# shaygong322/Mujoco-LIP-MPC-Simulation

Hardware: AMD Instinct MI355X
Metric: MPC solves/sec (batched scenarios), N=3 horizon 5-obstacle, 1->8 MI355X (higher is better)
Workload: dtype f64

## Files before the change

### mujoco-lip-mpc-simulation_amd/csrc/alipmpc.hip

```cpp
#include <hip/hip_runtime.h>

#include <atomic>
#include <cmath>
#include <cstdint>
#include <cstdio>
#include <cstdlib>
#include <cstring>
#include <map>
#include <mutex>
#include <string>
#include <type_traits>
#include <unordered_map>
#include <vector>

#include "../../include/alipmpc.h"

#ifndef ALIP_PART
#define ALIP_PART_HOST 1
#define ALIP_PART_N(k) 1
#else
#define ALIP_PART_HOST (ALIP_PART == 0)
#define ALIP_PART_N(k) (ALIP_PART == (k))
#endif

// ... 1534 lines not shown
#pragma unroll
        for (int q = 0; q < RPL; ++q) {
            const int r = lane + WAVE * q;
            if (r < mo4) {
                double* rq = rc + r;
                rq[0] = ck_put(sr[q]);
                rq[mo4] = ck_put(zl[q]);
                rq[2 * mo4] = ck_put(zu[q]);
                rq[3 * mo4] = ck_put(idl[q]);
                rq[4 * mo4] = ck_put(idu[q]);
                rq[5 * mo4] = ck_put(cr[q]);
                rq[6 * mo4] = ck_put(ra0[q]);
                rq[7 * mo4] = ck_put(ra1[q]);
#pragma unroll
                for (int i = 0; i < 4; ++i) rq[(8 + i) * mo4] = ck_put(rv[q][i]);
            }
        }
        double* rf = rc + ck_filt(mo4) + lane;
        if (lane < nf) {
            rf[0] = ck_put(fth0);
            rf[2 * WAVE] = ck_put(fph0);
        }
        if (lane + WAVE < nf) {
            rf[WAVE] = ck_put(fth1);
            rf[3 * WAVE] = ck_put(fph1);
        }
        if (lane < NG) rc[ck_vme(mo4) + lane] = ck_put(vme);
        const double sv[13] = {ck_put(mu), ck_put(f_cur), ck_put(lsum_cur), ck_put(theta_c), ck_put(dw_last),
                               (double)nf, (double)it, (double)n_rest, (double)fail_it, (double)it_end,
                               theta_ok ? 1.0 : 0.0, rp ? 1.0 : 0.0, ck_put(theta_R)};
        double v = 0.0;
#pragma unroll
        for (int i = 0; i < 13; ++i) v = lane == i ? sv[i] : v;
        if (lane < 13) rc[ck_scal(mo4) + lane] = v;
        if (lane == 0) P.cont[cont_hdr(P.B) + k] = (uint32_t)b;
        if constexpr (sizeof(R) == 8) {
            if (lane == 0 && !to_team) {
                const int cls = rp ? CONT_PEND : CONT_REG;
                P.cont[cont_list(P.B, cls, (long long)atomicAdd(P.cont + cls, 1u))] = (uint32_t)k;
            }
        }
    };
    R phi_R = R(0.0);
    it = it0;
    for (;;) {
    if constexpr (RS) {
        if (rpend) {
            rpend = false;
#ifndef ALIP_NO_SETPRIO
            if (PR && role == 2) __builtin_amdgcn_s_setprio(3);
#endif
            STAMP(8);
            RELANE();
#pragma unroll
            for (int q = 0; q < RPL; ++q) {
                const int r = lane + WAVE * q;
                if (r < mo4) {
                    w.ry[r] = sr[q];
                    w.rsig[r] = zl[q];
                    w.rw[r] = zu[q];
                }
            }
            if (lane < NG) w.V[lane] = vme;
            wave_sync();
            const int rr = rfl(resto_wave<N, KSM, R>(wv, fth0, fph0, fth1, fph1, nf, mu, theta_R, it));
            STAMP(25);
            const int rcode = rr & 15;
            it = rr >> 4;
            RELANE();
            vme = lane < NG ? w.V[lane] : R(0.0);
            R lr = R(0.0);
#pragma unroll
            for (int q = 0; q < RPL; ++q) {
                const int r = lane + WAVE * q;
                if (r < mo4) {
                    sr[q] = w.ry[r];
                    zl[q] = w.rsig[r];
                    zu[q] = w.rw[r];
                }
#pragma unroll
                for (int i = 0; i < 4; ++i) rv[q][i] = w.V[gen_i(rg[q], i)];
                R o[6];
#pragma unroll
                for (int i = 0; i < 6; ++i) o[i] = w.obs6[6 * roi[q] + i];
                row_trans(rtype[q], rv[q], w.cst[K_GXG], w.cst[K_GYG], ra0[q], ra1[q]);
                cr[q] = row_value(rtype[q], rk[q], rv[q], ra0[q], ra1[q], o, CK);
                const R d1 = sr[q] - cl[q], d2 = cu[q] - sr[q];
                lr += llog(HL(q) ? (HU(q) ? d1 * d2 : d1) : (HU(q) ? d2 : R(1.0)));
                idl[q] = HL(q) ? rcp_nr(d1) : R(0.0);
                idu[q] = HU(q) ? rcp_nr(d2) : R(0.0);
                zl[q] = HL(q) ? fmin(fmax(zl[q], mu * R(1e-10) * idl[q]), R(1e10) * mu * idl[q]) : R(0.0);
                zu[q] = HU(q) ? fmin(fmax(zu[q], mu * R(1e-10) * idu[q]), R(1e10) * mu * idu[q]) : R(0.0);
            }
            lsum_cur = wsum(lr);
            f_cur = obj_sum<N, RPL>(cr, mr4);
            theta_ok = false;
            wave_sync();
            STAMP(24);
            if (rcode == RSW_INFEASIBLE || rcode == RSW_FAILED) {
                status = 2;
                break;
            }
            if (rcode == RSW_MAXITER) break;
        }
    }
    for (; it <= max_iter; ++it) {
        if ((ckpt_it > 0 && it == ckpt_it) || (TM && ckpt_tr > 0 && w.cst[K_NTR] >= R(ckpt_tr))) {
            put_record(TM && !(ckpt_it > 0 && it == ckpt_it), false);
            status = ST_CKPT;
            break;
        }
#ifndef ALIP_NO_SETPRIO
        if ((TM && tm < 0) || (PR && (role == 1 || (role == 2 && n_rest > 0))))
            ;
        else if (PR && role == 2 && it == 20)
            ;
        else if (it == 8)
            __builtin_amdgcn_s_setprio(1);
        else if (it == 14)
            __builtin_amdgcn_s_setprio(2);
        else if (it == 20)
            __builtin_amdgcn_s_setprio(3);
#endif
        R gl[NT];
        R jv[JC ? KSM : 1][NT];
        for (;;) {
            RELANE();
#pragma unroll
            for (int q = 0; q < RPL; ++q) {
                const int r = lane + WAVE * q;
                R o[6], cf[4], hx[6];
#pragma unroll
                for (int i = 0; i < 6; ++i) o[i] = w.obs6[6 * roi[q] + i];
                row_coef(rtype[q], rk[q], rv[q], ra0[q], ra1[q], o, CK, cf, hx);
                if (r < mo4) {
                    st4(w.rcoef + 4 * r, cf[0], cf[1], cf[2], cf[3]);
                    w.ry[r] = rtype[q] == R_OBJ ? -R(1.0) : zl[q] - zu[q];
                }
                if (rtype[q] == R_VBX) {
                    w.CT[rk[q] + 1] = ra1[q];
                    w.ST[rk[q] + 1] = ra0[q];
                }
                if (rtype[q] == R_OBJ) {
#pragma unroll
                    for (int i = 0; i < 6; ++i) w.hobj[6 * rk[q] + i] = hx[i];
                }
            }
            wave_sync();
// ... 153 lines not shown
                const R* Gb = G + 8 * kb * NCP;
                R gv[NT], sgv[NT];
#ifdef ALIP_S_DENSE
                const unsigned SCOLS = 0xFFu;
#else
                const unsigned SCOLS = (s & 1) ? 0x7Fu : 0x73u;
#endif
#pragma unroll
                for (int T = 0; T < NT; ++T) {
                    gv[T] = G[t * NCP + 16 * T + col];
                    R a = R(0.0);
#pragma unroll
                    for (int c2 = 0; c2 < 8; ++c2)
                        if ((SCOLS >> c2) & 1u) a += Srow[c2] * Gb[c2 * NCP + 16 * T + col];
                    sgv[T] = a;
                }
                auto* a = acc[s & 1];
                a[0] = Mfma<R>::run(gv[0], sgv[0], a[0]);
                if constexpr (NT == 2) {
                    a[1] = Mfma<R>::run(gv[0], sgv[1], a[1]);
                    a[2] = Mfma<R>::run(gv[1], sgv[1], a[2]);
                }
            }
#pragma unroll
            for (int T = 0; T < NT; ++T) rhsc[T] = gsum(pw[T]);
#pragma unroll
            for (int i = 0; i < 4; ++i) {
                const int row = Mfma<R>::row(g4, i);
                w.K[row * KLD + col] = acc[0][0][i] + acc[1][0][i];
                if constexpr (NT == 2) {
                    const R k1 = acc[0][1][i] + acc[1][1][i];
                    w.K[row * KLD + 16 + col] = k1;
                    w.K[(16 + col) * KLD + row] = k1;
                    w.K[(16 + row) * KLD + 16 + col] = acc[0][2][i] + acc[1][2][i];
                }
            }
        }
        wave_sync();
        STAMP(4);
        RELANE();
        R xv;
        bool fact_ok = true;
        {
            R rhs_l = R(0.0);
#pragma unroll
            for (int T = 0; T < NT; ++T) rhs_l = (lane < n && (lane >> 4) == T) ? rhsc[T] : rhs_l;
            if constexpr (GJ && GJ_REGS) {
                R a[n + 1];
                auto fill = [&](R dw) {
#pragma unroll
                    for (int j = 0; j < n; ++j) a[j] = (lane < n ? w.K[lane * KLD + j] : R(0.0)) + (lane == j ? dw : R(0.0));
                    a[n] = rhs_l + R(0.0);
                };
                fill(R(0));
                if (!gj_regs<n, R, gj_rb<RPL>>(a, lane)) {
                    R dw = dw_last == R(0.0) ? R(1e-4) : fmax(R(1e-20), dw_last / R(3.0));
                    for (;;) {
                        fill(dw);
                        if (gj_regs<n, R, gj_rb<RPL>>(a, lane)) break;
                        dw *= dw_last == R(0.0) ? R(100.0) : R(8.0);
                        if (dw > R(sizeof(R) == 8 ? 1e40 : 1e30)) {
                            fact_ok = false;
                            break;
                        }
                    }
                    dw_last = uni(dw);
                }
                xv = lane < n ? a[n] : R(0.0);
            } else if constexpr (GJ) {
                if (lane < n) w.K[lane * KLD + n] = rhs_l;
                wave_sync();
                gj_fill<n, KLD, GJLD>(w.K, w.S, lane, R(0));
                wave_sync();
                if (!gj_lds<n, GJLD>(w.S, lane)) {
                    R dw = dw_last == R(0.0) ? R(1e-4) : fmax(R(1e-20), dw_last / R(3.0));
                    for (;;) {
                        gj_fill<n, KLD, GJLD>(w.K, w.S, lane, dw);
                        wave_sync();
                        if (gj_lds<n, GJLD>(w.S, lane)) break;
                        dw *= dw_last == R(0.0) ? R(100.0) : R(8.0);
                        if (dw > R(sizeof(R) == 8 ? 1e40 : 1e30)) {
                            fact_ok = false;
                            break;
                        }
                    }
                    dw_last = uni(dw);
                }
                xv = lane < n ? w.S[lane * GJLD + n] : R(0.0);
            } else {
                R a[n];
                R myidg = R(1.0);
#pragma unroll
                for (int j = 0; j < n; ++j) a[j] = lane < n ? w.K[lane * KLD + j] : (lane == j ? R(1.0) : R(0.0));
                if (!chol_rows<n>(a, myidg, lane)) {
                    R dw = dw_last == R(0.0) ? R(1e-4) : fmax(R(1e-20), dw_last / R(3.0));
                    for (;;) {
#pragma unroll
                        for (int j = 0; j < n; ++j)
                            a[j] = (lane < n ? w.K[lane * KLD + j] : (lane == j ? R(1.0) : R(0.0))) +
                                   (lane == j ? dw : R(0.0));
                        if (chol_rows<n>(a, myidg, lane)) break;
                        dw *= dw_last == R(0.0) ? R(100.0) : R(8.0);
                        if (dw > R(sizeof(R) == 8 ? 1e40 : 1e30)) {
                            fact_ok = false;
                            break;
                        }
                    }
                    dw_last = uni(dw);
                }
                R acc = R(0.0), yv = R(0.0);
#pragma unroll
                for (int k = 0; k < n; ++k) {
                    const R yk = bcast((rhs_l - acc) * myidg, k);
                    yv = lane == k ? yk : yv;
                    acc += lane > k ? a[k] * yk : R(0.0);
                }
                wave_sync();
                if (lane < n) {
#pragma unroll
// ... 3298 lines not shown
```

### mujoco-lip-mpc-simulation_amd/csrc/resto_wave.inc

```
enum { RSW_OK = 0, RSW_INFEASIBLE = 1, RSW_MAXITER = 2, RSW_FAILED = 3 };

template <int N, int KSM, class R>
__device__ __forceinline__ int resto_wave(int wv, R fth0, R fph0, R fth1, R fph1, int nfo, R mu_o, R theta_R, int it)
{
    using D = Dim<N>;
    constexpr int n = D::n;
    constexpr int NT = D::NT;
    constexpr int NCP = D::NCP;
    constexpr int NG = D::NG;
    constexpr int KLD = D::KLD;
    constexpr int RPL = (4 * KSM + WAVE - 1) / WAVE;
    extern __shared__ __attribute__((aligned(16))) double smem[];
    const KP& P = *reinterpret_cast<const KP*>(smem);
    const R* G = reinterpret_cast<const R*>(smem + KP_DOUBLES);
    R* wsb = const_cast<R*>(G) + NG * NCP;
    int lane = lane_id();
    RSTAMP_DECL
    const int mr4 = rfl(P.mr4), mo4 = rfl(P.mo4), m_max = rfl(P.m_max), rps = rfl(P.rps);
    const int nc_max = rfl(P.nc_max), ne_max = rfl(P.ne_max), nobs = nc_max + ne_max;
    const int modi = rfl(P.modi), max_iter = rfl(P.max_iter);
    WSS<N, R> w = carve_s<N, R>(wsb + (size_t)wv * wss_elems<N, R>(nc_max, ne_max, mr4, mo4), nc_max, ne_max, mr4, mo4);
    const int nc_sel = w.nsel[0], ne_sel = w.nsel[1];
    const R rho = R(1000.0), tol = w.cst[K_TOL];
    const R gth = R(1e-5), gph = R(1e-8), sth = R(1.1), sph = R(2.3), eta = R(1e-8), gal = R(0.05);
    int g4 = lane >> 4, col = lane & 15;
#define RS_RELANE()                                                                                               \
    do {                                                                                                          \
        RELAUNDER(lane);                                                                                          \
        g4 = lane >> 4;                                                                                           \
        col = lane & 15;                                                                                          \
        for (int q_ = 0; q_ < RPL; ++q_) {                                                                        \
            RELAUNDER(rtype[q_]);                                                                                 \
            RELAUNDER(rk[q_]);                                                                                    \
            RELAUNDER(roi[q_]);                                                                                   \
            RELAUNDER(rg[q_]);                                                                                    \
            RELAUNDER(cl[q_]);                                                                                    \
            RELAUNDER(cu[q_]);                                                                                    \
        }                                                                                                         \
    } while (0)
#define RCK load_rowk(w.cst)
    int rtype[RPL], rk[RPL], roi[RPL];
    uint32_t rg[RPL];
    R cl[RPL], cu[RPL], rv[RPL][4], rdv[RPL][4], ra0[RPL], ra1[RPL], cr[RPL];
    R sr[RPL], vl[RPL], vu[RPL], pp[RPL], nn[RPL], zp[RPL], zn[RPL], yv[RPL], s0[RPL], zl0[RPL], zu0[RPL];
    R mu = mu_o, nbl = R(0), mal = R(0);
#pragma unroll
    for (int q = 0; q < RPL; ++q) {
        const int r = lane + WAVE * q;
        RowInfo ri;
        ri.type = R_NONE; ri.k = 0; ri.slot = 0;
        if (r < m_max) {
            ri = decode_row(P, r, nc_sel, ne_sel);
        } else if (r >= mr4 && r < mr4 + N) {
            ri.type = R_OBJ;
            ri.k = r - mr4 + 1;
        }
        rtype[q] = ri.type;
        rk[q] = ri.k;
        roi[q] = ri.type == R_CIR ? ri.slot : (ri.type == R_ELP ? nc_max + ri.slot : 0);
        rg[q] = row_gens(ri.type, ri.k);
        const R clo = r < mr4 ? w.rclo[r] : R(-INFINITY), cuo = r < mr4 ? w.rcuo[r] : R(INFINITY);
        cl[q] = isfinite(clo) ? clo - R(1e-8) * fmax(R(1.0), fabs(clo)) : -INFINITY;
        cu[q] = isfinite(cuo) ? cuo + R(1e-8) * fmax(R(1.0), fabs(cuo)) : INFINITY;
        const bool isc = ri.type < R_NONE;
        sr[q] = r < mo4 && isc ? w.ry[r] : R(0);
        zl0[q] = r < mo4 && isc ? w.rsig[r] : R(0);
        zu0[q] = r < mo4 && isc ? w.rw[r] : R(0);
        s0[q] = sr[q];
#pragma unroll
        for (int i = 0; i < 4; ++i) {
            rv[q][i] = w.V[gen_i(rg[q], i)];
            rdv[q][i] = R(0);
        }
        R o[6];
#pragma unroll
        for (int i = 0; i < 6; ++i) o[i] = w.obs6[6 * roi[q] + i];
        row_trans(rtype[q], rv[q], w.cst[K_GXG], w.cst[K_GYG], ra0[q], ra1[q]);
        cr[q] = row_value(rtype[q], rk[q], rv[q], ra0[q], ra1[q], o, RCK);
        if (isc) {
            mu = fmax(mu, fabs(cr[q] - sr[q]));
            nbl += R(2) + (R)isfinite(cl[q]) + (R)isfinite(cu[q]);
            mal += R(1);
        }
    }
    mu = wmax(mu);
    nbl = wsum(nbl);
    mal = wsum(mal);
    const R xR = lane < n ? w.V[gp(lane / 3, lane % 3)] : R(0);
    const R d2 = lane < n ? R(1) / (fmax(R(1), fabs(xR)) * fmax(R(1), fabs(xR))) : R(0);
    R th0 = R(0);
#pragma unroll
    for (int q = 0; q < RPL; ++q) {
        const bool isc = rtype[q] < R_NONE;
        const R r_ = cr[q] - sr[q];
        const R a = (mu - rho * r_) / (R(2) * rho);
        const R sq = sqrt(a * a + mu * r_ / (R(2) * rho));
        const R nv = a >= R(0) ? a + sq : (mu * r_ / (R(2) * rho)) / (sq - a);
        nn[q] = isc ? nv : R(1);
        pp[q] = isc ? r_ + nv : R(1);
        zp[q] = isc ? mu / pp[q] : R(0);
        zn[q] = isc ? mu / nn[q] : R(0);
        vl[q] = isc && isfinite(cl[q]) ? fmin(rho, zl0[q]) : R(0);
        vu[q] = isc && isfinite(cu[q]) ? fmin(rho, zu0[q]) : R(0);
        yv[q] = R(0);
        if (isc) th0 += fabs(cr[q] - pp[q] + nn[q] - sr[q]);
    }
    th0 = wsum(th0);
    const R theta_max = R(1e4) * fmax(R(1), th0), theta_min = R(1e-4) * fmax(R(1), th0);
    R rft0 = INFINITY, rfp0 = INFINITY, rft1 = INFINITY, rfp1 = INFINITY;
    int nfr = 0;
    R dw_last = R(0);
    int code = RSW_OK;
    bool first = true;
    const int it_in = it;
    RSTAMP(0);
    for (;;) {
        RS_RELANE();
        R xc = lane < n ? w.V[gp(lane / 3, lane % 3)] : R(0);
        if (!first) {
            R tho = R(0), lso = R(0);
#pragma unroll
            for (int q = 0; q < RPL; ++q) {
                if (rtype[q] < R_NONE) tho += fabs(cr[q] - sr[q]);
                const R d1 = sr[q] - cl[q], d2_ = cu[q] - sr[q];
                lso += llog(isfinite(cl[q]) ? (isfinite(cu[q]) ? d1 * d2_ : d1) : (isfinite(cu[q]) ? d2_ : R(1.0)));
            }
            wsum_pair(tho, lso);
            const R fo = obj_sum<N, RPL>(cr, mr4);
            const R pho = fo - mu_o * lso;
            bool acc = isfinite(pho) && tho <= R(0.9) * theta_R;
            if (acc) {
                const bool b0 = lane < nfo && !(tho < fth0 || pho < fph0);
                const bool b1 = lane + WAVE < nfo && !(tho < fth1 || pho < fph1);
                acc = __ballot(b0 || b1) == 0ull;
            }
            if (acc) {
                const R tau = uni(fmax(R(0.99), R(1) - mu_o));
                R dzl[RPL], dzu[RPL], ad = R(1);
#pragma unroll
                for (int q = 0; q < RPL; ++q) {
                    const bool hl = rtype[q] < R_NONE && isfinite(cl[q]), hu = rtype[q] < R_NONE && isfinite(cu[q]);
                    const R e1 = s0[q] - cl[q], e2 = cu[q] - s0[q];
                    dzl[q] = hl ? mu_o / e1 - zl0[q] - zl0[q] / e1 * (sr[q] - s0[q]) : R(0);
                    dzu[q] = hu ? mu_o / e2 - zu0[q] + zu0[q] / e2 * (sr[q] - s0[q]) : R(0);
                    if (hl && dzl[q] < R(0)) ad = fmin(ad, -tau * zl0[q] / dzl[q]);
                    if (hu && dzu[q] < R(0)) ad = fmin(ad, -tau * zu0[q] / dzu[q]);
                }
                ad = wmin(ad);
                R zmax = R(0);
#pragma unroll
                for (int q = 0; q < RPL; ++q) {
                    zl0[q] += ad * dzl[q];
                    zu0[q] += ad * dzu[q];
                    zmax = fmax(zmax, fmax(zl0[q], zu0[q]));
                }
                zmax = wmax(zmax);
                if (zmax > R(1000)) {
#pragma unroll
                    for (int q = 0; q < RPL; ++q) {
                        zl0[q] = rtype[q] < R_NONE && isfinite(cl[q]) ? R(1) : R(0);
                        zu0[q] = rtype[q] < R_NONE && isfinite(cu[q]) ? R(1) : R(0);
                    }
                }
                code = RSW_OK;
                break;
            }
        }
        first = false;
        RSTAMP(1);
#pragma unroll
        for (int q = 0; q < RPL; ++q) {
            const int r = lane + WAVE * q;
            R o[6], cf[4], hx[6];
#pragma unroll
            for (int i = 0; i < 6; ++i) o[i] = w.obs6[6 * roi[q] + i];
            row_coef(rtype[q], rk[q], rv[q], ra0[q], ra1[q], o, RCK, cf, hx);
            if (r < mo4) {
                const bool isc = rtype[q] < R_NONE;
                st4(w.rcoef + 4 * r, isc ? cf[0] : R(0), isc ? cf[1] : R(0), isc ? cf[2] : R(0), isc ? cf[3] : R(0));
                w.ry[r] = isc ? yv[q] : R(0);
            }
            if (rtype[q] == R_VBX) {
                w.CT[rk[q] + 1] = ra1[q];
                w.ST[rk[q] + 1] = ra0[q];
            }
            if (rtype[q] == R_OBJ) {
#pragma unroll
                for (int i = 0; i < 6; ++i) w.hobj[6 * rk[q] + i] = R(0);
            }
        }
        wave_sync();
        constexpr bool JCR = KSM * NT <= 16;
        R jv[JCR ? KSM : 1][NT];
        R gl[NT];
#pragma unroll
        for (int T = 0; T < NT; ++T) gl[T] = R(0);
#pragma unroll
        for (int s = 0; s < KSM; ++s) {
            const int r = 4 * s + g4;
            const uint32_t pk = w.rgen[r];
            R ca0, ca1, cb0, cb1;
            ld4(w.rcoef + 4 * r, ca0, ca1, cb0, cb1);
            const R y = w.ry[r];
#pragma unroll
            for (int T = 0; T < NT; ++T) {
                const int cc = 16 * T + col;
                const R j = ca0 * G[gen_i(pk, 0) * NCP + cc] + ca1 * G[gen_i(pk, 1) * NCP + cc] +
                            cb0 * G[gen_i(pk, 2) * NCP + cc] + cb1 * G[gen_i(pk, 3) * NCP + cc];
                if constexpr (JCR) jv[JCR ? s : 0][T] = j;
                gl[T] += j * y;
            }
        }
#pragma unroll
        for (int T = 0; T < NT; ++T) gl[T] = gsum(gl[T]);
        R glme = gl[0];
#pragma unroll
        for (int T = 1; T < NT; ++T) glme = (lane >> 4) == T ? gl[T] : glme;
// ... 12 lines not shown
                nz += fabs(zp[q]) + fabs(zn[q]) + fabs(vl[q]) + fabs(vu[q]);
                whi = fmax(whi, fmax(pp[q] * zp[q], nn[q] * zn[q]));
                wlo = fmin(wlo, fmin(pp[q] * zp[q], nn[q] * zn[q]));
                if (isfinite(cl[q])) {
                    whi = fmax(whi, dl * vl[q]);
                    wlo = fmin(wlo, dl * vl[q]);
                }
                if (isfinite(cu[q])) {
                    whi = fmax(whi, du * vu[q]);
                    wlo = fmin(wlo, du * vu[q]);
                }
            }
        }
        wsum_pair(nz, ny);
        wmax_pair(dual, prim);
        wmaxmin_pair(whi, wlo);
        const R sd = uni(fmax(R(100), (nz + ny) / (R(n) + mal * R(3))) / R(100));
        const R sc = uni(fmax(R(100), nz / fmax(R(1), nbl)) / R(100));
        const R base = fmax(dual / sd, prim);
        const R e0 = uni(fmax(base, fmax(fabs(whi), fabs(wlo)) / sc));
        if (e0 <= tol) {
            R viol = R(0);
#pragma unroll
            for (int q = 0; q < RPL; ++q) {
                const int r = lane + WAVE * q;
                if (r < mr4 && rtype[q] < R_NONE) {
                    if (isfinite(cl[q])) viol = fmax(viol, w.rclo[r] - cr[q]);
                    if (isfinite(cu[q])) viol = fmax(viol, cr[q] - w.rcuo[r]);
                }
            }
            viol = wmax(viol);
            code = viol > R(1e-4) ? RSW_INFEASIBLE : RSW_OK;
            break;
        }
        if (it >= max_iter) {
            code = RSW_MAXITER;
            break;
        }
        const R mu_prev = mu;
        for (int t = 0; t < 8; ++t) {
            const R cm = fmax(fabs(whi - mu), fabs(wlo - mu));
            if (fmax(base, cm / sc) <= R(10) * mu && mu > tol / R(11))
                mu = uni(fmax(tol / R(11), fmin(R(0.2) * mu, mu * sqrt(mu))));
            else
                break;
        }
        if (mu != mu_prev) {
            nfr = 0;
            zeta = uni(sqrt(mu));
            gxv = lane < n ? zeta * d2 * (xc - xR) - glme : R(0);
        }
        const R tau = uni(fmax(R(0.99), R(1) - mu));
        RSTAMP(3);
        R iD[RPL], bv[RPL], iSp[RPL], iSn[RPL], iSs[RPL];
#pragma unroll
        for (int q = 0; q < RPL; ++q) {
            const int r = lane + WAVE * q;
            const bool isc = rtype[q] < R_NONE;
            const R dl = sr[q] - cl[q], du = cu[q] - sr[q];
            const R ipv = rcp_nr(pp[q]), inv = rcp_nr(nn[q]);
            const R idl_ = isfinite(cl[q]) ? rcp_nr(dl) : R(0), idu_ = isfinite(cu[q]) ? rcp_nr(du) : R(0);
            iSp[q] = isc ? pp[q] * rcp_nr(zp[q]) : R(0);
            iSn[q] = isc ? nn[q] * rcp_nr(zn[q]) : R(0);
            iSs[q] = isc ? rcp_nr(vl[q] * idl_ + vu[q] * idu_) : R(0);
            const R mdl = mu * idl_, mdu = mu * idu_;
            const R rc = cr[q] - pp[q] + nn[q] - sr[q];
            iD[q] = isc ? rcp_nr(iSp[q] + iSn[q] + iSs[q]) : R(0);
            bv[q] = isc ? -rc + (-rho - yv[q] + mu * ipv) * iSp[q] - (-rho + yv[q] + mu * inv) * iSn[q] +
                              (-yv[q] + mdl - mdu) * iSs[q]
                        : R(0);
            if (r < mo4) {
                w.rsig[r] = iD[q];
                w.rw[r] = isc ? yv[q] + bv[q] * iD[q] : R(0);
            }
        }
        wave_sync();
        RS_RELANE();
        RSTAMP(4);
        if constexpr (16 * (N + 1) <= WAVE)
            hess_blocks_lanes<N, R>(w, lane, rps, nobs, modi);
        else
            hess_blocks<N, R>(w, lane, rps, nobs, modi);
        wave_sync();
        RS_RELANE();
        RSTAMP(5);
        R rhsc[NT];
        {
            constexpr int NA = NT * (NT + 1) / 2;
            typename Mfma<R>::acc acc[2][NA];
#pragma unroll
            for (int h = 0; h < 2; ++h)
#pragma unroll
                for (int i = 0; i < NA; ++i) acc[h][i] = typename Mfma<R>::acc{R(0), R(0), R(0), R(0)};
            R pw[NT];
#pragma unroll
            for (int T = 0; T < NT; ++T) pw[T] = R(0);
#pragma unroll
            for (int s = 0; s < KSM; ++s) {
                const int r = 4 * s + g4;
                const R sg = w.rsig[r], wr = w.rw[r];
                R j[NT];
                if constexpr (JCR) {
#pragma unroll
                    for (int T = 0; T < NT; ++T) j[T] = jv[JCR ? s : 0][T];
                } else {
                    const uint32_t pk = w.rgen[r];
                    R ca0, ca1, cb0, cb1;
                    ld4(w.rcoef + 4 * r, ca0, ca1, cb0, cb1);
#pragma unroll
                    for (int T = 0; T < NT; ++T) {
                        const int cc = 16 * T + col;
                        j[T] = ca0 * G[gen_i(pk, 0) * NCP + cc] + ca1 * G[gen_i(pk, 1) * NCP + cc] +
                               cb0 * G[gen_i(pk, 2) * NCP + cc] + cb1 * G[gen_i(pk, 3) * NCP + cc];
                    }
                }
#pragma unroll
                for (int T = 0; T < NT; ++T) pw[T] += j[T] * wr;
                auto* a = acc[s & 1];
                a[0] = Mfma<R>::run(j[0], sg * j[0], a[0]);
                if constexpr (NT == 2) {
                    a[1] = Mfma<R>::run(j[0], sg * j[1], a[1]);
// ... 4 lines not shown
            for (int s = 1; s < NG / 4; ++s) {
                const int t = 4 * s + g4;
                const int kb = t >> 3;
                const R* Srow = w.S + 64 * kb + 8 * (t & 7);
                const R* Gb = G + 8 * kb * NCP;
                R gv[NT], sgv[NT];
                const unsigned SCOLS = (s & 1) ? 0x7Fu : 0x73u;
#pragma unroll
                for (int T = 0; T < NT; ++T) {
                    gv[T] = G[t * NCP + 16 * T + col];
                    R a = R(0);
#pragma unroll
                    for (int c2 = 0; c2 < 8; ++c2)
                        if ((SCOLS >> c2) & 1u) a += Srow[c2] * Gb[c2 * NCP + 16 * T + col];
                    sgv[T] = a;
                }
                auto* a = acc[s & 1];
                a[0] = Mfma<R>::run(gv[0], sgv[0], a[0]);
                if constexpr (NT == 2) {
                    a[1] = Mfma<R>::run(gv[0], sgv[1], a[1]);
                    a[2] = Mfma<R>::run(gv[1], sgv[1], a[2]);
                }
            }
#pragma unroll
            for (int T = 0; T < NT; ++T) rhsc[T] = gsum(pw[T]);
#pragma unroll
            for (int i = 0; i < 4; ++i) {
                const int row = Mfma<R>::row(g4, i);
                w.K[row * KLD + col] = acc[0][0][i] + acc[1][0][i];
                if constexpr (NT == 2) {
                    const R k1 = acc[0][1][i] + acc[1][1][i];
                    w.K[row * KLD + 16 + col] = k1;
                    w.K[(16 + col) * KLD + row] = k1;
                    w.K[(16 + row) * KLD + 16 + col] = acc[0][2][i] + acc[1][2][i];
                }
            }
        }
        wave_sync();
        if (lane < n) w.K[lane * KLD + lane] += zeta * d2;
        wave_sync();
        R rhs_l = R(0);
#pragma unroll
        for (int T = 0; T < NT; ++T) rhs_l = (lane < n && (lane >> 4) == T) ? rhsc[T] : rhs_l;
        rhs_l = lane < n ? rhs_l - zeta * d2 * (xc - xR) : R(0);
        RSTAMP(6);
        R xv;
        if constexpr (n <= ALIP_GJ_MAX_N) {
            R a[n + 1];
            auto fill = [&](R dw) {
#pragma unroll
                for (int j = 0; j < n; ++j) a[j] = (lane < n ? w.K[lane * KLD + j] : R(0)) + (lane == j ? dw : R(0));
                a[n] = rhs_l + R(0);
            };
            fill(R(0));
            bool ok = gj_regs<n, R, gj_rb<RPL>>(a, lane);
            if (!ok) {
                R dw = dw_last == R(0) ? R(1e-4) : fmax(R(1e-20), dw_last / R(3));
                for (;;) {
                    fill(dw);
                    if (gj_regs<n, R, gj_rb<RPL>>(a, lane)) {
                        ok = true;
                        break;
                    }
                    dw *= dw_last == R(0) ? R(100) : R(8);
                    if (dw > R(sizeof(R) == 8 ? 1e40 : 1e30)) break;
                }
                dw_last = uni(dw);
            }
            if (!ok) {
                code = RSW_FAILED;
                break;
            }
            xv = lane < n ? a[n] : R(0);
        } else {
            R a[n];
            R myidg = R(1);
#pragma unroll
            for (int j = 0; j < n; ++j) a[j] = lane < n ? w.K[lane * KLD + j] : (lane == j ? R(1) : R(0));
            bool ok = chol_rows<n>(a, myidg, lane);
            if (!ok) {
                R dw = dw_last == R(0) ? R(1e-4) : fmax(R(1e-20), dw_last / R(3));
                for (;;) {
#pragma unroll
                    for (int j = 0; j < n; ++j)
                        a[j] = (lane < n ? w.K[lane * KLD + j] : (lane == j ? R(1) : R(0))) + (lane == j ? dw : R(0));
                    if (chol_rows<n>(a, myidg, lane)) {
                        ok = true;
                        break;
                    }
                    dw *= dw_last == R(0) ? R(100) : R(8);
                    if (dw > R(sizeof(R) == 8 ? 1e40 : 1e30)) break;
                }
                dw_last = uni(dw);
            }
            if (!ok) {
                code = RSW_FAILED;
                break;
            }
            R acc = R(0), yy = R(0);
#pragma unroll
            for (int k = 0; k < n; ++k) {
                const R yk = bcast((rhs_l - acc) * myidg, k);
                yy = lane == k ? yk : yy;
                acc += lane > k ? a[k] * yk : R(0);
            }
            wave_sync();
            if (lane < n) {
#pragma unroll
                for (int j = 0; j < n; ++j) w.K[lane * KLD + j] = j <= lane ? a[j] : R(0);
            }
            wave_sync();
            acc = R(0);
            xv = R(0);
#pragma unroll
            for (int i = n - 1; i >= 0; --i) {
                const R xi = bcast((yy - acc) * myidg, i);
                xv = lane == i ? xi : xv;
                acc += lane < i ? w.K[i * KLD + (lane & 31)] * xi : R(0);
            }
        }
        RS_RELANE();
        RSTAMP(7);
        {
            R v = R(0);
            if constexpr (dp_rows<n, NG, R>) {
                v = gdp_rows<n, NCP>(G, xv, lane < NG ? lane : 0);
            } else {
#pragma unroll
                for (int j = 0; j < n; ++j) v += G[(lane < NG ? lane : 0) * NCP + j] * bcast(xv, j);
            }
            if (lane < NG) w.dV[lane] = v;
        }
        wave_sync();
        R dy[RPL], dpv[RPL], dnv[RPL], ds[RPL], dzp[RPL], dzn[RPL], dvl[RPL], dvu[RPL];
        R ap = R(1), az = R(1), theta = R(0), lin = R(0), gpn = R(0);
#pragma unroll
        for (int q = 0; q < RPL; ++q) {
            const int r = lane + WAVE * q;
#pragma unroll
            for (int i = 0; i < 4; ++i) rdv[q][i] = w.dV[gen_i(rg[q], i)];
            R jd = R(0);
            if (r < mo4) {
                R ca0, ca1, cb0, cb1;
                ld4(w.rcoef + 4 * r, ca0, ca1, cb0, cb1);
                jd = ca0 * rdv[q][0] + ca1 * rdv[q][1] + cb0 * rdv[q][2] + cb1 * rdv[q][3];
            }
            const bool isc = rtype[q] < R_NONE, hl = isc && isfinite(cl[q]), hu = isc && isfinite(cu[q]);
            const R dl = sr[q] - cl[q], du = cu[q] - sr[q];
            const R ipv = rcp_nr(pp[q]), inv = rcp_nr(nn[q]);
            const R idl_ = hl ? rcp_nr(dl) : R(0), idu_ = hu ? rcp_nr(du) : R(0);
            const R mdl = mu * idl_, mdu = mu * idu_;
            dy[q] = isc ? (bv[q] - jd) * iD[q] : R(0);
            dpv[q] = isc ? (-rho - yv[q] + mu * ipv - dy[q]) * iSp[q] : R(0);
            dnv[q] = isc ? (-rho + yv[q] + mu * inv + dy[q]) * iSn[q] : R(0);
            ds[q] = isc ? (-yv[q] + mdl - mdu - dy[q]) * iSs[q] : R(0);
            dzp[q] = isc ? mu * ipv - zp[q] - zp[q] * ipv * dpv[q] : R(0);
            dzn[q] = isc ? mu * inv - zn[q] - zn[q] * inv * dnv[q] : R(0);
            dvl[q] = hl ? mdl - vl[q] - vl[q] * idl_ * ds[q] : R(0);
            dvu[q] = hu ? mdu - vu[q] + vu[q] * idu_ * ds[q] : R(0);
            if (isc) {
                if (dpv[q] < R(0)) ap = fmin(ap, -tau * pp[q] * rcp_nr(dpv[q]));
                if (dnv[q] < R(0)) ap = fmin(ap, -tau * nn[q] * rcp_nr(dnv[q]));
                if (dzp[q] < R(0)) az = fmin(az, -tau * zp[q] * rcp_nr(dzp[q]));
                if (dzn[q] < R(0)) az = fmin(az, -tau * zn[q] * rcp_nr(dzn[q]));
                theta += fabs(cr[q] - pp[q] + nn[q] - sr[q]);
                gpn += (rho - mu * ipv) * dpv[q] + (rho - mu * inv) * dnv[q] - (mdl - mdu) * ds[q];
                lin += rho * (pp[q] + nn[q]) - mu * llog(pp[q] * nn[q] * (hl ? (hu ? dl * du : dl) : (hu ? du : R(1))));
            }
            const R ids = rcp_nr(ds[q]);
            if (hl && ds[q] < R(0)) ap = fmin(ap, -tau * dl * ids);
            if (hu && ds[q] > R(0)) ap = fmin(ap, tau * du * ids);
            if (hl && dvl[q] < R(0)) az = fmin(az, -tau * vl[q] * rcp_nr(dvl[q]));
            if (hu && dvu[q] < R(0)) az = fmin(az, -tau * vu[q] * rcp_nr(dvu[q]));
        }
        const R ex = lane < n ? xc - xR : R(0);
        lin += R(0.5) * zeta * d2 * ex * ex;
        gpn += zeta * d2 * ex * xv;
        wmin_pair(ap, az);
        wsum_pair(theta, gpn);
        const R gphi = gpn;
        const R phi = wsum(lin);
        R amin;
        if (gphi < R(0)) {
            amin = fmin(gth, gph * theta / -gphi);
            if (theta <= theta_min) amin = fmin(amin, exp(sth * llog(theta) - sph * llog(-gphi)));
        } else {
            amin = gth;
        }
        amin *= gal;
        amin = uni(amin > R(0) ? amin : R(8.673617379884035e-19));
        RSTAMP(8);
        R al = ap;
        bool accepted = false, ftype = false;
        R ctr[RPL], ta0[RPL], ta1[RPL];
        const R dxl = lane < n ? xv : R(0);
        while (al >= amin) {
            R tht = R(0), lt = R(0);
            bool bad = false;
#pragma unroll
            for (int q = 0; q < RPL; ++q) {
                R vt[4];
#pragma unroll
                for (int i = 0; i < 4; ++i) vt[i] = fma(al, rdv[q][i], rv[q][i]);
                R o[6];
#pragma unroll
                for (int i = 0; i < 6; ++i) o[i] = w.obs6[6 * roi[q] + i];
                row_trans(rtype[q], vt, w.cst[K_GXG], w.cst[K_GYG], ta0[q], ta1[q]);
                ctr[q] = row_value(rtype[q], rk[q], vt, ta0[q], ta1[q], o, RCK);
                if (rtype[q] < R_NONE) {
                    const R pt = pp[q] + al * dpv[q], nt = nn[q] + al * dnv[q], st = sr[q] + al * ds[q];
                    tht += fabs(ctr[q] - pt + nt - st);
                    const R d1 = st - cl[q], d2_ = cu[q] - st;
                    if (!(pt > R(0)) || !(nt > R(0))) bad = true;
                    if (isfinite(cl[q]) && !(d1 > R(0))) bad = true;
                    if (isfinite(cu[q]) && !(d2_ > R(0))) bad = true;
                    lt += rho * (pt + nt) -
                          mu * llog(pt * nt * (isfinite(cl[q]) ? (isfinite(cu[q]) ? d1 * d2_ : d1)
                                                               : (isfinite(cu[q]) ? d2_ : R(1))));
                }
// ... 25 lines not shown
                    ftype = false;
                }
            }
            if (accepted) break;
            al = uni(al * R(0.5));
        }
        RSTAMP(9);
        if (!accepted) {
            code = RSW_FAILED;
            break;
        }
        if (!ftype && nfr < FILTER_CAP) {
            const R fvt = (R(1) - gth) * theta, fvp = phi - gph * theta;
            if ((nfr & (WAVE - 1)) == lane) {
                if (nfr < WAVE) {
                    rft0 = fvt;
                    rfp0 = fvp;
                } else {
                    rft1 = fvt;
                    rfp1 = fvp;
                }
            }
            nfr++;
        }
        if (lane < NG) w.V[lane] = fma(al, w.dV[lane], w.V[lane]);
#pragma unroll
        for (int q = 0; q < RPL; ++q) {
#pragma unroll
            for (int i = 0; i < 4; ++i) rv[q][i] = fma(al, rdv[q][i], rv[q][i]);
            ra0[q] = ta0[q];
            ra1[q] = ta1[q];
            cr[q] = ctr[q];
            if (rtype[q] < R_NONE) {
                pp[q] += al * dpv[q];
                nn[q] += al * dnv[q];
                sr[q] += al * ds[q];
                yv[q] += al * dy[q];
                zp[q] += az * dzp[q];
                zn[q] += az * dzn[q];
                vl[q] += az * dvl[q];
                vu[q] += az * dvu[q];
                const R ks = R(1e10);
                zp[q] = fmin(fmax(zp[q], mu / (ks * pp[q])), ks * mu / pp[q]);
                zn[q] = fmin(fmax(zn[q], mu / (ks * nn[q])), ks * mu / nn[q]);
                const R d1 = sr[q] - cl[q], d2_ = cu[q] - sr[q];
                vl[q] = isfinite(cl[q]) ? fmin(fmax(vl[q], mu / (ks * d1)), ks * mu / d1) : R(0);
                vu[q] = isfinite(cu[q]) ? fmin(fmax(vu[q], mu / (ks * d2_)), ks * mu / d2_) : R(0);
            }
        }
        wave_sync();
        ++it;
        RSTAMP(10);
    }
    wave_sync();
#pragma unroll
    for (int q = 0; q < RPL; ++q) {
        const int r = lane + WAVE * q;
        if (r < mo4) {
            w.ry[r] = sr[q];
            w.rsig[r] = zl0[q];
            w.rw[r] = zu0[q];
        }
    }
    wave_sync();
    RSTAMP(11);
    RSTAMP_FLUSH(it - it_in);
    return (it << 4) | code;
#undef RS_RELANE
#undef RCK
}
```

Measured before the change: 7.835 million.

## Pass restoration row state in registers instead of round-tripping through LDS

The restoration-phase routine now takes the caller's per-row register arrays (types, bounds, slacks, multipliers, constraint values) by reference. This drops the LDS write-back and re-read of slacks and multipliers and the row decoding and constraint evaluation it repeated on entry. On a successful return it also hands back the barrier-log sum and objective, so the caller skips recomputing them. It also reuses reciprocals computed in the matrix build for the step direction, makes the acceptance test compute the log-barrier only when the theta test passes, and merges the regularised factorisation retry into one loop, at the cost of higher register pressure in the inlined routine.

Measured after the change: 7.942 million (median of 6 runs). +1.4%, better.

```diff
diff --git a/mujoco-lip-mpc-simulation_amd/csrc/alipmpc.hip b/mujoco-lip-mpc-simulation_amd/csrc/alipmpc.hip
--- a/mujoco-lip-mpc-simulation_amd/csrc/alipmpc.hip
+++ b/mujoco-lip-mpc-simulation_amd/csrc/alipmpc.hip
@@ -1610,48 +1610,44 @@
 #endif
             STAMP(8);
             RELANE();
-#pragma unroll
-            for (int q = 0; q < RPL; ++q) {
-                const int r = lane + WAVE * q;
-                if (r < mo4) {
-                    w.ry[r] = sr[q];
-                    w.rsig[r] = zl[q];
-                    w.rw[r] = zu[q];
-                }
-            }
             if (lane < NG) w.V[lane] = vme;
             wave_sync();
-            const int rr = rfl(resto_wave<N, KSM, R>(wv, fth0, fph0, fth1, fph1, nf, mu, theta_R, it));
+            R lso = R(0.0), fro = R(0.0);
+            const int rr = rfl(resto_wave<N, KSM, R>(wv, fth0, fph0, fth1, fph1, nf, mu, theta_R, it, rtype, rk, roi, rg,
+                                                     cl, cu, rv, ra0, ra1, cr, sr, zl, zu, lso, fro));
             STAMP(25);
             const int rcode = rr & 15;
             it = rr >> 4;
             RELANE();
             vme = lane < NG ? w.V[lane] : R(0.0);
-            R lr = R(0.0);
+            if (rcode == RSW_OK_ORIG) {
+                lsum_cur = lso;
+                f_cur = fro;
+            } else {
+                R lr = R(0.0);
+#pragma unroll
+                for (int q = 0; q < RPL; ++q) {
+#pragma unroll
+                    for (int i = 0; i < 4; ++i) rv[q][i] = w.V[gen_i(rg[q], i)];
+                    R o[6];
+#pragma unroll
+                    for (int i = 0; i < 6; ++i) o[i] = w.obs6[6 * roi[q] + i];
+                    row_trans(rtype[q], rv[q], w.cst[K_GXG], w.cst[K_GYG], ra0[q], ra1[q]);
+                    cr[q] = row_value(rtype[q], rk[q], rv[q], ra0[q], ra1[q], o, CK);
+                    const R d1 = sr[q] - cl[q], d2 = cu[q] - sr[q];
+                    lr += llog(HL(q) ? (HU(q) ? d1 * d2 : d1) : (HU(q) ? d2 : R(1.0)));
+                }
+                lsum_cur = wsum(lr);
+                f_cur = obj_sum<N, RPL>(cr, mr4);
+            }
 #pragma unroll
             for (int q = 0; q < RPL; ++q) {
-                const int r = lane + WAVE * q;
-                if (r < mo4) {
-                    sr[q] = w.ry[r];
-                    zl[q] = w.rsig[r];
-                    zu[q] = w.rw[r];
-                }
-#pragma unroll
-                for (int i = 0; i < 4; ++i) rv[q][i] = w.V[gen_i(rg[q], i)];
-                R o[6];
-#pragma unroll
-                for (int i = 0; i < 6; ++i) o[i] = w.obs6[6 * roi[q] + i];
-                row_trans(rtype[q], rv[q], w.cst[K_GXG], w.cst[K_GYG], ra0[q], ra1[q]);
-                cr[q] = row_value(rtype[q], rk[q], rv[q], ra0[q], ra1[q], o, CK);
                 const R d1 = sr[q] - cl[q], d2 = cu[q] - sr[q];
-                lr += llog(HL(q) ? (HU(q) ? d1 * d2 : d1) : (HU(q) ? d2 : R(1.0)));
                 idl[q] = HL(q) ? rcp_nr(d1) : R(0.0);
                 idu[q] = HU(q) ? rcp_nr(d2) : R(0.0);
                 zl[q] = HL(q) ? fmin(fmax(zl[q], mu * R(1e-10) * idl[q]), R(1e10) * mu * idl[q]) : R(0.0);
                 zu[q] = HU(q) ? fmin(fmax(zu[q], mu * R(1e-10) * idu[q]), R(1e10) * mu * idu[q]) : R(0.0);
             }
-            lsum_cur = wsum(lr);
-            f_cur = obj_sum<N, RPL>(cr, mr4);
             theta_ok = false;
             wave_sync();
             STAMP(24);
@@ -1911,6 +1907,23 @@
                     for (int j = 0; j < n; ++j) a[j] = (lane < n ? w.K[lane * KLD + j] : R(0.0)) + (lane == j ? dw : R(0.0));
                     a[n] = rhs_l + R(0.0);
                 };
+                if constexpr (RS) {
+                    R dw = R(0);
+                    for (;;) {
+                        fill(dw);
+                        if (gj_regs<n, R, gj_rb<RPL>>(a, lane)) break;
+                        if (dw == R(0)) {
+                            dw = dw_last == R(0.0) ? R(1e-4) : fmax(R(1e-20), dw_last / R(3.0));
+                        } else {
+                            dw *= dw_last == R(0.0) ? R(100.0) : R(8.0);
+                            if (dw > R(sizeof(R) == 8 ? 1e40 : 1e30)) {
+                                fact_ok = false;
+                                break;
+                            }
+                        }
+                    }
+                    if (dw != R(0)) dw_last = uni(dw);
+                } else {
                 fill(R(0));
                 if (!gj_regs<n, R, gj_rb<RPL>>(a, lane)) {
                     R dw = dw_last == R(0.0) ? R(1e-4) : fmax(R(1e-20), dw_last / R(3.0));
@@ -1924,6 +1937,7 @@
                         }
                     }
                     dw_last = uni(dw);
+                }
                 }
                 xv = lane < n ? a[n] : R(0.0);
             } else if constexpr (GJ) {
diff --git a/mujoco-lip-mpc-simulation_amd/csrc/resto_wave.inc b/mujoco-lip-mpc-simulation_amd/csrc/resto_wave.inc
--- a/mujoco-lip-mpc-simulation_amd/csrc/resto_wave.inc
+++ b/mujoco-lip-mpc-simulation_amd/csrc/resto_wave.inc
@@ -1,26 +1,28 @@
-enum { RSW_OK = 0, RSW_INFEASIBLE = 1, RSW_MAXITER = 2, RSW_FAILED = 3 };
+enum { RSW_OK = 0, RSW_INFEASIBLE = 1, RSW_MAXITER = 2, RSW_FAILED = 3, RSW_OK_ORIG = 4 };
 
-template <int N, int KSM, class R>
-__device__ __forceinline__ int resto_wave(int wv, R fth0, R fph0, R fth1, R fph1, int nfo, R mu_o, R theta_R, int it)
+template <int N, int KSM, class R, int RPL>
+__device__ __forceinline__ int resto_wave(int wv, R fth0, R fph0, R fth1, R fph1, int nfo, R mu_o, R theta_R, int it,
+                                          int (&rtype)[RPL], int (&rk)[RPL], int (&roi)[RPL], uint32_t (&rg)[RPL],
+                                          R (&cl)[RPL], R (&cu)[RPL], R (&rv)[RPL][4], R (&ra0)[RPL], R (&ra1)[RPL],
+                                          R (&cr)[RPL], R (&sr)[RPL], R (&zl0)[RPL], R (&zu0)[RPL], R& lsum_o, R& f_o)
 {
+    static_assert(RPL == (4 * KSM + WAVE - 1) / WAVE, "one row group per 64 rows");
     using D = Dim<N>;
     constexpr int n = D::n;
     constexpr int NT = D::NT;
     constexpr int NCP = D::NCP;
     constexpr int NG = D::NG;
     constexpr int KLD = D::KLD;
-    constexpr int RPL = (4 * KSM + WAVE - 1) / WAVE;
     extern __shared__ __attribute__((aligned(16))) double smem[];
     const KP& P = *reinterpret_cast<const KP*>(smem);
     const R* G = reinterpret_cast<const R*>(smem + KP_DOUBLES);
     R* wsb = const_cast<R*>(G) + NG * NCP;
     int lane = lane_id();
     RSTAMP_DECL
-    const int mr4 = rfl(P.mr4), mo4 = rfl(P.mo4), m_max = rfl(P.m_max), rps = rfl(P.rps);
+    const int mr4 = rfl(P.mr4), mo4 = rfl(P.mo4), rps = rfl(P.rps);
     const int nc_max = rfl(P.nc_max), ne_max = rfl(P.ne_max), nobs = nc_max + ne_max;
     const int modi = rfl(P.modi), max_iter = rfl(P.max_iter);
     WSS<N, R> w = carve_s<N, R>(wsb + (size_t)wv * wss_elems<N, R>(nc_max, ne_max, mr4, mo4), nc_max, ne_max, mr4, mo4);
-    const int nc_sel = w.nsel[0], ne_sel = w.nsel[1];
     const R rho = R(1000.0), tol = w.cst[K_TOL];
     const R gth = R(1e-5), gph = R(1e-8), sth = R(1.1), sph = R(2.3), eta = R(1e-8), gal = R(0.05);
     int g4 = lane >> 4, col = lane & 15;
@@ -39,53 +41,18 @@
         }                                                                                                         \
     } while (0)
 #define RCK load_rowk(w.cst)
-    int rtype[RPL], rk[RPL], roi[RPL];
-    uint32_t rg[RPL];
-    R cl[RPL], cu[RPL], rv[RPL][4], rdv[RPL][4], ra0[RPL], ra1[RPL], cr[RPL];
-    R sr[RPL], vl[RPL], vu[RPL], pp[RPL], nn[RPL], zp[RPL], zn[RPL], yv[RPL], s0[RPL], zl0[RPL], zu0[RPL];
-    R mu = mu_o, nbl = R(0), mal = R(0);
+    R rdv[RPL][4];
+    R vl[RPL], vu[RPL], pp[RPL], nn[RPL], zp[RPL], zn[RPL], yv[RPL], s0[RPL];
+    const R mal = w.cst[K_MACT], nbl = R(2) * mal + w.cst[K_NBL];
+    R mu = mu_o;
 #pragma unroll
     for (int q = 0; q < RPL; ++q) {
-        const int r = lane + WAVE * q;
-        RowInfo ri;
-        ri.type = R_NONE; ri.k = 0; ri.slot = 0;
-        if (r < m_max) {
-            ri = decode_row(P, r, nc_sel, ne_sel);
-        } else if (r >= mr4 && r < mr4 + N) {
-            ri.type = R_OBJ;
-            ri.k = r - mr4 + 1;
-        }
-        rtype[q] = ri.type;
-        rk[q] = ri.k;
-        roi[q] = ri.type == R_CIR ? ri.slot : (ri.type == R_ELP ? nc_max + ri.slot : 0);
-        rg[q] = row_gens(ri.type, ri.k);
-        const R clo = r < mr4 ? w.rclo[r] : R(-INFINITY), cuo = r < mr4 ? w.rcuo[r] : R(INFINITY);
-        cl[q] = isfinite(clo) ? clo - R(1e-8) * fmax(R(1.0), fabs(clo)) : -INFINITY;
-        cu[q] = isfinite(cuo) ? cuo + R(1e-8) * fmax(R(1.0), fabs(cuo)) : INFINITY;
-        const bool isc = ri.type < R_NONE;
-        sr[q] = r < mo4 && isc ? w.ry[r] : R(0);
-        zl0[q] = r < mo4 && isc ? w.rsig[r] : R(0);
-        zu0[q] = r < mo4 && isc ? w.rw[r] : R(0);
         s0[q] = sr[q];
 #pragma unroll
-        for (int i = 0; i < 4; ++i) {
-            rv[q][i] = w.V[gen_i(rg[q], i)];
-            rdv[q][i] = R(0);
-        }
-        R o[6];
-#pragma unroll
-        for (int i = 0; i < 6; ++i) o[i] = w.obs6[6 * roi[q] + i];
-        row_trans(rtype[q], rv[q], w.cst[K_GXG], w.cst[K_GYG], ra0[q], ra1[q]);
-        cr[q] = row_value(rtype[q], rk[q], rv[q], ra0[q], ra1[q], o, RCK);
-        if (isc) {
-            mu = fmax(mu, fabs(cr[q] - sr[q]));
-            nbl += R(2) + (R)isfinite(cl[q]) + (R)isfinite(cu[q]);
-            mal += R(1);
-        }
+        for (int i = 0; i < 4; ++i) rdv[q][i] = R(0);
+        if (rtype[q] < R_NONE) mu = fmax(mu, fabs(cr[q] - sr[q]));
     }
     mu = wmax(mu);
-    nbl = wsum(nbl);
-    mal = wsum(mal);
     const R xR = lane < n ? w.V[gp(lane / 3, lane % 3)] : R(0);
     const R d2 = lane < n ? R(1) / (fmax(R(1), fabs(xR)) * fmax(R(1), fabs(xR))) : R(0);
     R th0 = R(0);
@@ -118,21 +85,30 @@
         RS_RELANE();
         R xc = lane < n ? w.V[gp(lane / 3, lane % 3)] : R(0);
         if (!first) {
-            R tho = R(0), lso = R(0);
-#pragma unroll
-            for (int q = 0; q < RPL; ++q) {
+            R tho = R(0);
+#pragma unroll
+            for (int q = 0; q < RPL; ++q)
                 if (rtype[q] < R_NONE) tho += fabs(cr[q] - sr[q]);
-                const R d1 = sr[q] - cl[q], d2_ = cu[q] - sr[q];
-                lso += llog(isfinite(cl[q]) ? (isfinite(cu[q]) ? d1 * d2_ : d1) : (isfinite(cu[q]) ? d2_ : R(1.0)));
-            }
-            wsum_pair(tho, lso);
-            const R fo = obj_sum<N, RPL>(cr, mr4);
-            const R pho = fo - mu_o * lso;
-            bool acc = isfinite(pho) && tho <= R(0.9) * theta_R;
+            tho = wsum(tho);
+            bool acc = tho <= R(0.9) * theta_R;
             if (acc) {
-                const bool b0 = lane < nfo && !(tho < fth0 || pho < fph0);
-                const bool b1 = lane + WAVE < nfo && !(tho < fth1 || pho < fph1);
-                acc = __ballot(b0 || b1) == 0ull;
+                R lso = R(0);
+#pragma unroll
+                for (int q = 0; q < RPL; ++q) {
+                    const R d1 = sr[q] - cl[q], d2_ = cu[q] - sr[q];
+                    lso += llog(isfinite(cl[q]) ? (isfinite(cu[q]) ? d1 * d2_ : d1) : (isfinite(cu[q]) ? d2_ : R(1.0)));
+                }
+                lso = wsum(lso);
+                const R fo = obj_sum<N, RPL>(cr, mr4);
+                const R pho = fo - mu_o * lso;
+                lsum_o = lso;
+                f_o = fo;
+                acc = isfinite(pho);
+                if (acc) {
+                    const bool b0 = lane < nfo && !(tho < fth0 || pho < fph0);
+                    const bool b1 = lane + WAVE < nfo && !(tho < fth1 || pho < fph1);
+                    acc = __ballot(b0 || b1) == 0ull;
+                }
             }
             if (acc) {
                 const R tau = uni(fmax(R(0.99), R(1) - mu_o));
@@ -162,7 +138,7 @@
                         zu0[q] = rtype[q] < R_NONE && isfinite(cu[q]) ? R(1) : R(0);
                     }
                 }
-                code = RSW_OK;
+                code = RSW_OK_ORIG;
                 break;
             }
         }
@@ -281,21 +257,23 @@
         }
         const R tau = uni(fmax(R(0.99), R(1) - mu));
         RSTAMP(3);
-        R iD[RPL], bv[RPL], iSp[RPL], iSn[RPL], iSs[RPL];
+        R iD[RPL], bv[RPL], iSp[RPL], iSn[RPL], iSs[RPL], ipv[RPL], inv[RPL], idl_[RPL], idu_[RPL];
 #pragma unroll
         for (int q = 0; q < RPL; ++q) {
             const int r = lane + WAVE * q;
             const bool isc = rtype[q] < R_NONE;
             const R dl = sr[q] - cl[q], du = cu[q] - sr[q];
-            const R ipv = rcp_nr(pp[q]), inv = rcp_nr(nn[q]);
-            const R idl_ = isfinite(cl[q]) ? rcp_nr(dl) : R(0), idu_ = isfinite(cu[q]) ? rcp_nr(du) : R(0);
+            ipv[q] = rcp_nr(pp[q]);
+            inv[q] = rcp_nr(nn[q]);
+            idl_[q] = isfinite(cl[q]) ? rcp_nr(dl) : R(0);
+            idu_[q] = isfinite(cu[q]) ? rcp_nr(du) : R(0);
             iSp[q] = isc ? pp[q] * rcp_nr(zp[q]) : R(0);
             iSn[q] = isc ? nn[q] * rcp_nr(zn[q]) : R(0);
-            iSs[q] = isc ? rcp_nr(vl[q] * idl_ + vu[q] * idu_) : R(0);
-            const R mdl = mu * idl_, mdu = mu * idu_;
+            iSs[q] = isc ? rcp_nr(vl[q] * idl_[q] + vu[q] * idu_[q]) : R(0);
+            const R mdl = mu * idl_[q], mdu = mu * idu_[q];
             const R rc = cr[q] - pp[q] + nn[q] - sr[q];
             iD[q] = isc ? rcp_nr(iSp[q] + iSn[q] + iSs[q]) : R(0);
-            bv[q] = isc ? -rc + (-rho - yv[q] + mu * ipv) * iSp[q] - (-rho + yv[q] + mu * inv) * iSn[q] +
+            bv[q] = isc ? -rc + (-rho - yv[q] + mu * ipv[q]) * iSp[q] - (-rho + yv[q] + mu * inv[q]) * iSn[q] +
                               (-yv[q] + mdl - mdu) * iSs[q]
                         : R(0);
             if (r < mo4) {
@@ -406,21 +384,20 @@
                 for (int j = 0; j < n; ++j) a[j] = (lane < n ? w.K[lane * KLD + j] : R(0)) + (lane == j ? dw : R(0));
                 a[n] = rhs_l + R(0);
             };
-            fill(R(0));
-            bool ok = gj_regs<n, R, gj_rb<RPL>>(a, lane);
-            if (!ok) {
-                R dw = dw_last == R(0) ? R(1e-4) : fmax(R(1e-20), dw_last / R(3));
-                for (;;) {
-                    fill(dw);
-                    if (gj_regs<n, R, gj_rb<RPL>>(a, lane)) {
-                        ok = true;
-                        break;
-                    }
+            R dw = R(0);
+            bool ok;
+            for (;;) {
+                fill(dw);
+                ok = gj_regs<n, R, gj_rb<RPL>>(a, lane);
+                if (ok) break;
+                if (dw == R(0)) {
+                    dw = dw_last == R(0) ? R(1e-4) : fmax(R(1e-20), dw_last / R(3));
+                } else {
                     dw *= dw_last == R(0) ? R(100) : R(8);
                     if (dw > R(sizeof(R) == 8 ? 1e40 : 1e30)) break;
                 }
-                dw_last = uni(dw);
-            }
+            }
+            if (dw != R(0)) dw_last = uni(dw);
             if (!ok) {
                 code = RSW_FAILED;
                 break;
@@ -429,24 +406,24 @@
         } else {
             R a[n];
             R myidg = R(1);
-#pragma unroll
-            for (int j = 0; j < n; ++j) a[j] = lane < n ? w.K[lane * KLD + j] : (lane == j ? R(1) : R(0));
-            bool ok = chol_rows<n>(a, myidg, lane);
-            if (!ok) {
-                R dw = dw_last == R(0) ? R(1e-4) : fmax(R(1e-20), dw_last / R(3));
-                for (;;) {
-#pragma unroll
-                    for (int j = 0; j < n; ++j)
-                        a[j] = (lane < n ? w.K[lane * KLD + j] : (lane == j ? R(1) : R(0))) + (lane == j ? dw : R(0));
-                    if (chol_rows<n>(a, myidg, lane)) {
-                        ok = true;
-                        break;
-                    }
+            R dw = R(0);
+            bool ok;
+            for (;;) {
+#pragma unroll
+                for (int j = 0; j < n; ++j) {
+                    const R kv = lane < n ? w.K[lane * KLD + j] : (lane == j ? R(1) : R(0));
+                    a[j] = dw == R(0) ? kv : kv + (lane == j ? dw : R(0));
+                }
+                ok = chol_rows<n>(a, myidg, lane);
+                if (ok) break;
+                if (dw == R(0)) {
+                    dw = dw_last == R(0) ? R(1e-4) : fmax(R(1e-20), dw_last / R(3));
+                } else {
                     dw *= dw_last == R(0) ? R(100) : R(8);
                     if (dw > R(sizeof(R) == 8 ? 1e40 : 1e30)) break;
                 }
-                dw_last = uni(dw);
-            }
+            }
+            if (dw != R(0)) dw_last = uni(dw);
             if (!ok) {
                 code = RSW_FAILED;
                 break;
@@ -501,24 +478,22 @@
             }
             const bool isc = rtype[q] < R_NONE, hl = isc && isfinite(cl[q]), hu = isc && isfinite(cu[q]);
             const R dl = sr[q] - cl[q], du = cu[q] - sr[q];
-            const R ipv = rcp_nr(pp[q]), inv = rcp_nr(nn[q]);
-            const R idl_ = hl ? rcp_nr(dl) : R(0), idu_ = hu ? rcp_nr(du) : R(0);
-            const R mdl = mu * idl_, mdu = mu * idu_;
+            const R mdl = mu * idl_[q], mdu = mu * idu_[q];
             dy[q] = isc ? (bv[q] - jd) * iD[q] : R(0);
-            dpv[q] = isc ? (-rho - yv[q] + mu * ipv - dy[q]) * iSp[q] : R(0);
-            dnv[q] = isc ? (-rho + yv[q] + mu * inv + dy[q]) * iSn[q] : R(0);
+            dpv[q] = isc ? (-rho - yv[q] + mu * ipv[q] - dy[q]) * iSp[q] : R(0);
+            dnv[q] = isc ? (-rho + yv[q] + mu * inv[q] + dy[q]) * iSn[q] : R(0);
             ds[q] = isc ? (-yv[q] + mdl - mdu - dy[q]) * iSs[q] : R(0);
-            dzp[q] = isc ? mu * ipv - zp[q] - zp[q] * ipv * dpv[q] : R(0);
-            dzn[q] = isc ? mu * inv - zn[q] - zn[q] * inv * dnv[q] : R(0);
-            dvl[q] = hl ? mdl - vl[q] - vl[q] * idl_ * ds[q] : R(0);
-            dvu[q] = hu ? mdu - vu[q] + vu[q] * idu_ * ds[q] : R(0);
+            dzp[q] = isc ? mu * ipv[q] - zp[q] - zp[q] * ipv[q] * dpv[q] : R(0);
+            dzn[q] = isc ? mu * inv[q] - zn[q] - zn[q] * inv[q] * dnv[q] : R(0);
+            dvl[q] = hl ? mdl - vl[q] - vl[q] * idl_[q] * ds[q] : R(0);
+            dvu[q] = hu ? mdu - vu[q] + vu[q] * idu_[q] * ds[q] : R(0);
             if (isc) {
                 if (dpv[q] < R(0)) ap = fmin(ap, -tau * pp[q] * rcp_nr(dpv[q]));
                 if (dnv[q] < R(0)) ap = fmin(ap, -tau * nn[q] * rcp_nr(dnv[q]));
                 if (dzp[q] < R(0)) az = fmin(az, -tau * zp[q] * rcp_nr(dzp[q]));
                 if (dzn[q] < R(0)) az = fmin(az, -tau * zn[q] * rcp_nr(dzn[q]));
                 theta += fabs(cr[q] - pp[q] + nn[q] - sr[q]);
-                gpn += (rho - mu * ipv) * dpv[q] + (rho - mu * inv) * dnv[q] - (mdl - mdu) * ds[q];
+                gpn += (rho - mu * ipv[q]) * dpv[q] + (rho - mu * inv[q]) * dnv[q] - (mdl - mdu) * ds[q];
                 lin += rho * (pp[q] + nn[q]) - mu * llog(pp[q] * nn[q] * (hl ? (hu ? dl * du : dl) : (hu ? du : R(1))));
             }
             const R ids = rcp_nr(ds[q]);
@@ -650,17 +625,6 @@
         ++it;
         RSTAMP(10);
     }
-    wave_sync();
-#pragma unroll
-    for (int q = 0; q < RPL; ++q) {
-        const int r = lane + WAVE * q;
-        if (r < mo4) {
-            w.ry[r] = sr[q];
-            w.rsig[r] = zl0[q];
-            w.rw[r] = zu0[q];
-        }
-    }
-    wave_sync();
     RSTAMP(11);
     RSTAMP_FLUSH(it - it_in);
     return (it << 4) | code;
```
